# uncbiag/DeepAtlas

Hardware: AMD Instinct MI355X
Metric: training volumes/sec at 160x192x160 fp32; Dice vs CPU ref (higher is better)
Workload: dtype f32; 1 GPU; seg-only UNet_light + softmax-Dice + Adam training step, batch 2/GPU, 160x192x160 fp32 (BASELINE configs[1]); global_batch=2, n_classes=32, parallelism=dp1, matrix_precision=fp32_split, hip_graph=False, matrix_arithmetic_bits=22

## Files before the change

deepatlas_amd/_native.py:

```python
import ctypes
import os
from ctypes import c_int, c_float, c_double, c_longlong, c_size_t, c_void_p, c_char_p, POINTER

import torch

_HERE = os.path.dirname(os.path.abspath(__file__))
LIB_PATH = os.environ.get('DA_LIB') or os.path.join(_HERE, 'csrc', 'libdeepatlas_hip.so')

P = c_void_p
I = c_int
F = c_float
LL = c_longlong
SZ = c_size_t
DBL = c_double

SIGNATURES = {
    'da_version': (I, []),
    'da_device_info': (I, [POINTER(c_int), POINTER(c_int), POINTER(c_size_t), c_char_p, I]),
    'da_w_oik_to_tio': (I, [P, P, I, I, I, P]),
    'da_w_tio_to_oik': (I, [P, P, I, I, I, P]),
    'da_w_iok_to_tio': (I, [P, P, I, I, I, P]),
    'da_w_tio_to_iok': (I, [P, P, I, I, I, P]),
    'da_w_iok_flip_to_tio': (I, [P, P, I, I, I, P]),
    'da_w_tio_to_iok_flip': (I, [P, P, I, I, I, P]),
    'da_w_tio_to_oik_acc': (I, [P, P, I, I, I, P]),
    'da_w_tio_to_iok_acc': (I, [P, P, I, I, I, P]),
    'da_w_tio_to_iok_flip_acc': (I, [P, P, I, I, I, P]),
    'da_conv3d_k3_ws_bytes': (SZ, [I, I, I, I, I, I, I]),
    'da_conv3d_k3_pack_bytes': (SZ, [I, I, I, I, I, I]),
    'da_conv3d_k3_dgrad_bst': (I, [P, P, P, I, P, I, I, I, I, I, I, P, P, F, P, I, P, P, SZ, P]),
    'da_conv3d_k3_prepack': (I, [P, I, I, I, I, I, I, I, I, P, SZ, P, SZ, P, P]),
    'da_conv3d_k3_use_prepacked': (None, [P, P, SZ, P, SZ]),
    'da_conv3d_k3_prepack_many': (I, [I, P, P, P, P, P, P, P, P, P, P, P, P, P, P, P]),
    'da_conv3d_k3_fwd': (I, [P, I, P, I, P, P, P, I, I, I, I, I, I, F, P, SZ, P]),
    'da_conv3d_k3_fwd_bnstats': (I, [P, I, P, I, P, P, P, I, I, I, I, I, I, P, I, POINTER(c_int), P, SZ, P]),
    'da_conv3d_k3_dgrad': (I, [P, P, P, I, P, I, I, I, I, I, I, I, P, SZ, P]),
    'da_conv3d_k3_wgrad': (I, [P, I, P, I, P, P, P, I, I, I, I, I, I, P, SZ, P]),
    'da_conv3d_k3_fwd_pro': (I, [P, I, P, P, F, P, I, P, P, F, P, P, P, I, I, I, I, I, F, P, I, POINTER(c_int), P, SZ, P]),
    'da_conv3d_k3_wgrad_pro': (I, [P, I, P, P, F, P, I, P, P, F, P, P, I, I, I, I, I, P, SZ, P]),
    'da_upconv3d_k3_supported': (I, [I, I, I]),
    'da_upconv3d_k3_ws_bytes': (SZ, [I, I, I, I, I, I]),
    'da_upconv3d_k3_fwd': (I, [P, I, P, I, P, P, P, I, I, I, I, I, F, P, SZ, P]),
    'da_upconv3d_k3_dgrad': (I, [P, P, P, I, P, I, I, I, I, I, I, P, SZ, P]),
    'da_upconv3d_k3_wgrad': (I, [P, I, P, I, P, P, I, I, I, I, I, P, SZ, P]),
    'da_set_conv_direct': (I, [I]),
    'da_set_matrix_bf16': (I, [I]),
    'da_set_matrix_mode': (I, [I]),
    'da_pointwise_ws_bytes': (SZ, [I, I, I]),
    'da_conv1x1_fwd': (I, [P, P, P, P, LL, I, I, P, SZ, P]),
    'da_conv1x1_fwd_pro': (I, [P, P, P, F, P, P, P, LL, I, I, P, SZ, P]),
    'da_conv1x1_wgrad_pro': (I, [P, P, P, F, P, P, P, LL, I, I, P, SZ, P]),
    'da_conv1x1_dgrad': (I, [P, P, P, LL, I, I, P, SZ, P]),
    'da_conv1x1_wgrad_ws_bytes': (SZ, [LL, I, I]),
    'da_conv1x1_wgrad': (I, [P, P, P, P, LL, I, I, P, SZ, P]),
    'da_deconv_k2s2_fwd': (I, [P, P, P, P, I, I, I, I, I, I, P, SZ, P]),
    'da_deconv_k2s2_fwd_bnstats': (I, [P, P, P, P, I, I, I, I, I, I, P, I, POINTER(c_int), P, SZ, P]),
    'da_deconv_k2s2_dgrad': (I, [P, P, P, I, I, I, I, I, I, P, SZ, P]),
    'da_deconv_k2s2_bn_bwd_ws_bytes': (SZ, [I, I, I, I, I, I]),
    'da_deconv_k2s2_bn_bwd': (I, [P, P, P, P, P, P, F, P, P, P, P, P, P, P, I, I, I, I, I, I, P, I, P, SZ, P]),
    'da_deconv_k2s2_wgrad_ws_bytes': (SZ, [I, I, I, I, I, I]),
    'da_deconv_k2s2_wgrad': (I, [P, P, P, P, I, I, I, I, I, I, P, SZ, P]),
    'da_bn_ws_bytes': (SZ, [LL, I]),
    'da_bn_train_stats': (I, [P, LL, I, P, P, F, F, P, P, P, P, P, P, P, SZ, P]),
    'da_bn_train_stats_from_partials': (I, [P, I, LL, I, P, P, F, F, P, P, P, P, P, P, P]),
    'da_bn_eval_affine': (I, [P, P, P, P, F, I, P, P, P, P, P]),
    'da_bn_act_fwd': (I, [P, P, P, F, P, LL, I, P]),
    'da_bn_act_bwd': (I, [P, P, P, P, P, P, P, F, I, P, P, P, LL, I, P, SZ, P]),
    'da_bn_act_bwd_dbias': (I, [P, P, P, P, P, P, F, I, P, P, P, P, LL, I, P, SZ, P]),
    'da_bn_act_bwd_dbias_pre': (I, [P, P, P, P, P, P, F, I, P, P, P, P, LL, I, P, I, P, SZ, P]),
    'da_act_bwd': (I, [P, P, F, P, LL, P]),
    'da_act_bwd_add_dbias': (I, [P, P, P, F, P, P, LL, I, P, SZ, P]),
    'da_colsum': (I, [P, LL, I, P, P, SZ, P]),
    'da_act_bwd_add_partial': (I, [P, P, P, F, P, LL, I, P, SZ, POINTER(c_int), P]),
    'da_colsum_finish': (I, [P, I, I, P, I, P]),
    'da_maxpool2_fwd': (I, [P, P, I, I, I, I, I, P]),
    'da_maxpool2_fwd_pro': (I, [P, P, P, F, P, P, I, I, I, I, I, P]),
    'da_maxpool2_bwd': (I, [P, P, P, I, I, I, I, I, P]),
    'da_maxpool2_bwd_add': (I, [P, P, P, P, I, I, I, I, I, P]),
    'da_maxpool2_bwd_bst': (I, [P, P, P, P, I, I, I, I, I, P, F, P, I, P, P]),
    'da_upsample_nearest_fwd': (I, [P, P, I, I, I, I, I, I, I, I, P]),
    'da_upsample_nearest_bwd': (I, [P, P, I, I, I, I, I, I, I, I, P]),
    'da_warp_fwd': (I, [P, P, P, P, I, I, I, I, I, P]),
    'da_warp_bwd': (I, [P, P, P, P, P, I, I, I, I, I, P]),
    'da_label_warp_dice_ws_bytes': (SZ, [I, I]),
    'da_warp_dice_ws_bytes': (SZ, [I, I]),
    'da_warp_dice_fwd': (I, [P, P, P, I, I, I, I, I, I, I, I, F, P, P, P, SZ, P]),
    'da_softmax_dice_fwd': (I, [P, P, I, P, I, LL, I, I, I, F, P, P, P, SZ, P]),
    'da_label_warp_dice_fwd': (I, [P, I, P, I, P, I, I, I, I, I, I, I, F, P, P, P, SZ, P]),
    'da_label_warp_dice_bwd': (I, [P, I, P, I, P, P, P, P, I, I, I, I, I, P]),
    'da_softwarp_dice_ws_bytes': (SZ, [I, I]),
    'da_softwarp_dice_fwd': (I, [P, I, P, P, I, I, I, I, I, I, I, I, F, P, P, P, SZ, P]),
    'da_softwarp_dice_bwd_disp': (I, [P, I, P, P, P, P, P, I, I, I, I, I, P]),
    'da_softwarp_dice_bwd_logits': (I, [P, I, P, P, P, P, P, I, I, I, I, I, P]),
    'da_warp_adjoint_labels': (I, [P, I, P, P, P, I, I, I, I, I, P]),
    'da_seg_anat_dlogits': (I, [P, P, I, P, P, P, P, P, P, P, I, LL, I, P]),
    'da_warp_bwd_dsrc_det_ws_bytes': (SZ, [I, I, I, I, I]),
    'da_warp_bwd_dsrc_det': (I, [P, P, P, I, I, I, I, I, P, SZ, P]),
    'da_identity_grid': (I, [P, I, I, I, I, P]),
    'da_warp_labels_fwd': (I, [P, I, P, P, I, I, I, I, I, P]),
    'da_warp_labels_bwd': (I, [P, P, I, P, P, I, I, I, I, I, P]),
    'da_dice_ws_bytes': (SZ, [I, LL, I]),
    'da_dice_fwd': (I, [P, P, I, P, I, LL, I, I, I, I, F, P, P, P, SZ, P]),
    'da_dice_bwd': (I, [P, P, I, P, P, P, P, I, LL, I, I, P]),
    'da_softmax_fwd': (I, [P, P, LL, I, P]),
    'da_softmax_bwd': (I, [P, P, P, LL, I, P]),
    'da_one_hot': (I, [P, I, P, LL, I, P]),
    'da_head_dice_ws_bytes': (SZ, [I, LL, I, I]),
    'da_head_dice_fwd': (I, [P, P, P, F, P, P, P, I, I, LL, I, I, I, I, F, P, P, P, SZ, P]),
    'da_head_dice_bwd': (I, [P, P, P, F, P, P, P, I, P, P, P, P, P, I, LL, I, I, P, SZ, P]),
    'da_head_dice_bwd_bst': (I, [P, P, P, F, P, P, P, P, I, P, P, P, P, P, I, LL, I, I, P, I, P, P, SZ, P]),
# ... 218 lines not shown
```

deepatlas_amd/csrc/deconv.hip:

```cpp
#include "common.h"
#include "pointwise_internal.h"

namespace {

template <int CT>
__global__ void __launch_bounds__(256)
deconv_k2s2_fwd_kernel(const float* __restrict__ in, const float* __restrict__ w, const float* __restrict__ bias,
                       float* __restrict__ out, int N, int D, int H, int W, int Cin, int Cout) {
    const long long nvox = (long long)N * D * H * W;
    const long long v = (long long)blockIdx.x * blockDim.x + threadIdx.x;
    if (v >= nvox) return;
    const int co0 = blockIdx.y * CT;
    long long r = v;
    const int iw = (int)(r % W); r /= W;
    const int ih = (int)(r % H); r /= H;
    const int id = (int)(r % D); const int n = (int)(r / D);
    const float* x = in + v * Cin;
    const int Ho = 2 * H, Wo = 2 * W, Do = 2 * D;
#pragma unroll 1
    for (int ij = 0; ij < 4; ++ij) {
        const int i = ij >> 1, j = ij & 1;
        float acc[2][CT];
#pragma unroll
        for (int k = 0; k < 2; ++k)
// ... 153 lines not shown
static int parts_for(long long units, int O, long long* per) {
    long long parts = units < 1024 ? units : 1024;
    const long long cap = (long long)(64ull << 20) / ((long long)O * 4);
    if (parts > cap) parts = cap;
    if (parts < 1) parts = 1;
    *per = da_cdiv(units, parts);
    return (int)da_cdiv(units, *per);
}

}

extern "C" size_t da_pointwise_ws_bytes(int ntaps, int Cin, int Cout) { return da_pw_packed_bytes(ntaps, Cin, Cout) + 256; }

extern "C" int da_deconv_k2s2_fwd(const float* in, const float* w_tio, const float* bias, float* out,
                                  int N, int D, int H, int W, int Cin, int Cout, void* ws, size_t ws_bytes, void* stream) {
    if (!in || !w_tio || !out || N <= 0 || D <= 0 || H <= 0 || W <= 0 || Cin <= 0 || Cout <= 0) return DA_ERR_BADARG;
    const long long nvox = (long long)N * D * H * W;
    if (da_pw_supported(Cin, Cout))
        return da_pw_gemm(in, w_tio, 0, bias, out, nvox, D, H, W, Cin, Cout, 8, 1, 0, ws, ws_bytes, da_stream(stream));
    hipLaunchKernelGGL((deconv_k2s2_fwd_kernel<16>), dim3((unsigned)da_cdiv(nvox, 256), (unsigned)da_cdiv(Cout, 16)), dim3(256), 0, da_stream(stream),
                       in, w_tio, bias, out, N, D, H, W, Cin, Cout);
    DA_LAUNCH_CHECK();
    return 0;
}

extern "C" int da_deconv_k2s2_fwd_bnstats(const float* in, const float* w_tio, const float* bias, float* out,
                                          int N, int D, int H, int W, int Cin, int Cout,
                                          double* stats_partial, int stats_capacity, int* stats_nparts,
                                          void* ws, size_t ws_bytes, void* stream) {
    if (stats_nparts) *stats_nparts = 0;
    if (!in || !w_tio || !out || N <= 0 || D <= 0 || H <= 0 || W <= 0 || Cin <= 0 || Cout <= 0) return DA_ERR_BADARG;
    const long long nvox = (long long)N * D * H * W;
    const long long nblk = da_cdiv(nvox, 256);
    if (stats_partial && stats_nparts && da_pw_supported(Cin, Cout) && nblk <= stats_capacity) {
        const int rc = da_pw_gemm(in, w_tio, 0, bias, out, nvox, D, H, W, Cin, Cout, 8, 1, 0, ws, ws_bytes, da_stream(stream), stats_partial);
        if (rc == 0) *stats_nparts = (int)nblk;
        return rc;
    }
    return da_deconv_k2s2_fwd(in, w_tio, bias, out, N, D, H, W, Cin, Cout, ws, ws_bytes, stream);
}

extern "C" int da_deconv_k2s2_dgrad(const float* dy, const float* w_tio, float* dx,
                                    int N, int D, int H, int W, int Cin, int Cout, void* ws, size_t ws_bytes, void* stream) {
    if (!dy || !w_tio || !dx || N <= 0 || D <= 0 || H <= 0 || W <= 0 || Cin <= 0 || Cout <= 0) return DA_ERR_BADARG;
    const long long nvox = (long long)N * D * H * W;
    if (da_pw_supported(Cout, Cin))
        return da_pw_gemm(dy, w_tio, 1, nullptr, dx, nvox, D, H, W, Cout, Cin, 8, 1, 1, ws, ws_bytes, da_stream(stream));
    hipLaunchKernelGGL((deconv_k2s2_dgrad_kernel<16>), dim3((unsigned)da_cdiv(nvox, 256), (unsigned)da_cdiv(Cin, 16)), dim3(256), 0, da_stream(stream),
                       dy, w_tio, dx, N, D, H, W, Cin, Cout);
    DA_LAUNCH_CHECK();
    return 0;
}

struct BnBwdWs { size_t bn_bytes, fused_bytes; void *bn, *fused; size_t bytes; };
static BnBwdWs bn_bwd_layout(long long M, int Cin, int Cout, void* ws) {
    const size_t bn = da_bn_ws_bytes(M * 8, Cout), fused = da_deconv_bn_bwd_ws_bytes(M, Cin, Cout);
    DaCarve c(ws); return BnBwdWs{bn, fused, c.take<char>(bn), c.take<char>(fused), c.off};
}
extern "C" size_t da_deconv_k2s2_bn_bwd_ws_bytes(int N, int D, int H, int W, int Cin, int Cout) {
    return bn_bwd_layout((long long)N * D * H * W, Cin, Cout, nullptr).bytes;
}
extern "C" int da_deconv_k2s2_bn_bwd(const float* gout, const float* y, const float* mean, const float* rstd, const float* scale, const float* shift, float act_slope,
                                     const float* in, const float* w_tio, float* dx, float* dw_tio, float* dbias, float* dgamma, float* dbeta,
                                     int N, int D, int H, int W, int Cin, int Cout, const double* pre, int pre_n,
                                     void* ws, size_t ws_bytes, void* stream) {
    if (!gout || !y || !mean || !rstd || !scale || !shift || !in || !w_tio || !dx || !dw_tio || N <= 0 || D <= 0 || H <= 0 || W <= 0) return DA_ERR_BADARG;
    if (!da_deconv_bn_bwd_supported(Cin, Cout)) return DA_ERR_UNSUPPORTED;
    if (ws_bytes < da_deconv_k2s2_bn_bwd_ws_bytes(N, D, H, W, Cin, Cout)) return DA_ERR_WS_SMALL;
    const long long M = (long long)N * D * H * W;
    hipStream_t st = da_stream(stream);
    const BnBwdWs l = bn_bwd_layout(M, Cin, Cout, ws);
    const float* cm = nullptr;
    int rc = da_bn_bwd_sums(gout, y, mean, rstd, scale, shift, act_slope, M * 8, Cout, dgamma, dbeta, &cm, l.bn, l.bn_bytes, st, pre, pre_n);
    if (rc) return rc;
    return da_deconv_bn_bwd(gout, y, mean, rstd, scale, shift, cm, act_slope, in, w_tio, dx, dw_tio, dbias, M, D, H, W, Cin, Cout, l.fused, l.fused_bytes, st);
}

constexpr size_t kWgPad = 512;
static size_t wgrad_bytes(size_t direct_floats, size_t matrix_bytes, int Cout) {
    const size_t direct = da_align(direct_floats * sizeof(float));
    return (direct > matrix_bytes ? direct : matrix_bytes) + kWgPad + da_bn_ws_bytes(0, Cout);
}
static size_t k2s2_wgrad_bytes(int N, int D, int H, int W, int Cin, int Cout, int Cbias) {
    long long per;
    const int O = 8 * Cin * Cout;
    const int parts = parts_for((long long)N * D * H * W, O, &per);
    const size_t mf = da_pw_supported(Cin, Cout) ? da_pw_wgrad_ws_bytes((long long)N * D * H * W, 8, Cin, Cout) : 0;
    return wgrad_bytes((size_t)parts * O, mf, Cbias);
}
extern "C" size_t da_deconv_k2s2_wgrad_ws_bytes(int N, int D, int H, int W, int Cin, int Cout) { return k2s2_wgrad_bytes(N, D, H, W, Cin, Cout, Cout); }

extern "C" int da_deconv_k2s2_wgrad(const float* in, const float* dy, float* dw_tio, float* dbias,
                                    int N, int D, int H, int W, int Cin, int Cout,
                                    void* ws, size_t ws_bytes, void* stream) {
    if (!in || !dy || !dw_tio || N <= 0 || D <= 0 || H <= 0 || W <= 0 || Cin <= 0 || Cout <= 0) return DA_ERR_BADARG;
    if (ws_bytes < da_deconv_k2s2_wgrad_ws_bytes(N, D, H, W, Cin, Cout)) return DA_ERR_WS_SMALL;
    hipStream_t st = da_stream(stream);
    long long per;
    const int O = 8 * Cin * Cout;
    const int parts = parts_for((long long)N * D * H * W, O, &per);
    const DaColsumTail cs = da_colsum_tail(ws, da_deconv_k2s2_wgrad_ws_bytes(N, D, H, W, Cin, Cout), Cout);
    int rc_pw = DA_ERR_UNSUPPORTED;
    if (da_pw_supported(Cin, Cout)) rc_pw = da_pw_wgrad(in, dy, dw_tio, (long long)N * D * H * W, D, H, W, Cin, Cout, 8, 1, ws, cs.front, st);
    if (rc_pw != 0 && rc_pw != DA_ERR_UNSUPPORTED) return rc_pw;
    if (rc_pw == DA_ERR_UNSUPPORTED) {
        float* partial = (float*)ws;
// ... 203 lines not shown
```

deepatlas_amd/csrc/pointwise_internal.h:

```cpp
#pragma once
#include <hip/hip_runtime.h>
#include <stddef.h>

bool da_pw_supported(int K, int N);
size_t da_pw_packed_bytes(int ntaps, int K, int N);
int da_pw_gemm(const float* a, const float* w, int transposed, const float* bias, float* out,
               long long M, int D, int H, int W, int K, int N, int ntaps, int up, int gather,
               void* ws, size_t ws_bytes, hipStream_t st, double* stats_partial = nullptr,
               const float* pro_scale = nullptr, const float* pro_shift = nullptr, float pro_slope = -1.f,
               int a_bf16 = 0, int out_bf16 = 0);
size_t da_pw_wgrad_ws_bytes(long long M, int ntaps, int Cin, int Cout);
int da_pw_wgrad(const float* in, const float* dy, float* dw, long long M, int D, int H, int W, int Cin, int Cout,
                int ntaps, int up, void* ws, size_t ws_bytes, hipStream_t st,
                const float* pro_scale = nullptr, const float* pro_shift = nullptr, float pro_slope = -1.f, int in_bf16 = 0, int dy_bf16 = 0);

int da_bn_bwd_sums(const float* dy, const float* x, const float* mean, const float* rstd, const float* scale, const float* shift, float act_slope,
                   long long M, int C, float* dgamma, float* dbeta, const float** cm_out, void* ws, size_t ws_bytes, hipStream_t st, const double* pre, int pre_n);
bool da_deconv_bn_bwd_supported(int Cin, int Cout);
size_t da_deconv_bn_bwd_ws_bytes(long long M, int Cin, int Cout);
int da_deconv_bn_bwd(const float* gout, const float* y, const float* mean, const float* rstd, const float* scale, const float* shift, const float* cm, float slope,
                     const float* in, const float* w_tio, float* dx, float* dw_tio, float* dbias,
                     long long M, int D, int H, int W, int Cin, int Cout, void* ws, size_t ws_bytes, hipStream_t st);
```

deepatlas_amd/csrc/pointwise_mfma.hip:

```cpp
#include "common.h"
#include "pointwise_internal.h"

typedef float f32x4 __attribute__((ext_vector_type(4)));

namespace {

struct PwP {
    const float* a; const float* wp; const float* bias; float* out;
    long long M;
    int D, H, W;
    int K, Nc;
    int lda, ldo;
    int accum;
    int ntaps, up;
    double* stats; int stats_ld;
    const float* ps; const float* pt; float pslope;
};

__device__ __forceinline__ float pw_act01(float z, float s) { return fmaxf(z, z * s); }

__device__ __forceinline__ long long fine0(long long v, int D, int H, int W) {
    int n, d, h, w; da_vox4(v, D, H, W, n, d, h, w);
    return (((long long)n * (2 * D) + 2 * d) * (2 * H) + 2 * h) * (long long)(2 * W) + 2 * w;
}
__device__ __forceinline__ long long tapoff(int t, int H, int W) {
    return ((long long)(t >> 2) * (2 * H) + ((t >> 1) & 1)) * (2 * W) + (t & 1);
}

template <int KC, int NT, bool GATHER, bool STATS = false, typename TA = float, typename TO = float>
__global__ void __launch_bounds__(256) pw_mfma_kernel(PwP p) {
    static_assert(!(STATS && GATHER), "statistics are an epilogue of the scatter form");
    const TA* __restrict__ pa = reinterpret_cast<const TA*>(p.a);
    TO* __restrict__ po = reinterpret_cast<TO*>(p.out);
    constexpr int MT = 4;
    const int lane = threadIdx.x & 63;
    const int wave = threadIdx.x >> 6;
    const int i = lane & 15, g = lane >> 4;
    const long long vbase = ((long long)blockIdx.x * 4 + wave) * (MT * 16);
    if (!STATS && vbase >= p.M) return;
    double d1[STATS ? NT : 1], d2[STATS ? NT : 1];
#pragma unroll
    for (int n = 0; n < (STATS ? NT : 1); ++n) { d1[n] = 0.0; d2[n] = 0.0; }
    const float4* wp4 = reinterpret_cast<const float4*>(p.wp) + lane;

    long long arow[MT];
    bool aval[MT];
#pragma unroll
    for (int r = 0; r < MT; ++r) {
        const long long v = vbase + r * 16 + i;
        aval[r] = v < p.M;
        const long long vv = aval[r] ? v : 0;
        arow[r] = (GATHER && p.up) ? fine0(vv, p.D, p.H, p.W) : vv;
    }
    f32x4 acc[MT][NT];

    if constexpr (!GATHER) {
        float4 a[MT][KC];
#pragma unroll
        for (int r = 0; r < MT; ++r)
#pragma unroll
            for (int c = 0; c < KC; ++c)
                a[r][c] = aval[r] ? da_ldq(pa, (arow[r] * p.lda + 16 * c + 4 * g) >> 2) : make_float4(0.f, 0.f, 0.f, 0.f);
        if (p.ps) {
#pragma unroll
            for (int c = 0; c < KC; ++c) {
                const float4 sc = *reinterpret_cast<const float4*>(p.ps + 16 * c + 4 * g), sf = *reinterpret_cast<const float4*>(p.pt + 16 * c + 4 * g);
#pragma unroll
                for (int r = 0; r < MT; ++r) {
                    a[r][c].x = pw_act01(a[r][c].x * sc.x + sf.x, p.pslope); a[r][c].y = pw_act01(a[r][c].y * sc.y + sf.y, p.pslope);
                    a[r][c].z = pw_act01(a[r][c].z * sc.z + sf.z, p.pslope); a[r][c].w = pw_act01(a[r][c].w * sc.w + sf.w, p.pslope);
                    if constexpr (DaEl<TA>::bf) a[r][c] = da_unpack_bf16x4(da_pack_bf16x4(a[r][c]));
                }
            }
        }
        long long orow[MT][4];
#pragma unroll
        for (int r = 0; r < MT; ++r)
#pragma unroll
            for (int reg = 0; reg < 4; ++reg) {
                const long long v = vbase + r * 16 + 4 * g + reg;
                orow[r][reg] = (v < p.M) ? (p.up ? fine0(v, p.D, p.H, p.W) : v) : -1;
            }
        long long obase[MT][4];
#pragma unroll
        for (int r = 0; r < MT; ++r)
#pragma unroll
            for (int reg = 0; reg < 4; ++reg) obase[r][reg] = orow[r][reg] * p.ldo + i;
        float bv[NT];
#pragma unroll
        for (int n = 0; n < NT; ++n) bv[n] = (p.bias && !p.accum) ? p.bias[16 * n + i] : 0.f;
#pragma unroll 1
        for (int t = 0; t < p.ntaps; ++t) {
            const long long toff = p.up ? tapoff(t, p.H, p.W) : 0;
#pragma unroll
            for (int r = 0; r < MT; ++r)
#pragma unroll
                for (int n = 0; n < NT; ++n) acc[r][n] = (f32x4){bv[n], bv[n], bv[n], bv[n]};
            if (p.accum) {
#pragma unroll
                for (int r = 0; r < MT; ++r)
#pragma unroll
                    for (int reg = 0; reg < 4; ++reg) {
                        if (orow[r][reg] < 0) continue;
                        const long long o = (orow[r][reg] + toff) * p.ldo + i;
#pragma unroll
                        for (int n = 0; n < NT; ++n) acc[r][n][reg] = da_ld1(po, o + 16 * n);
                    }
// ... 5 lines not shown
                    const float4 b = wp4[(((size_t)t * NT + n) * KC + c) * 64];
#pragma unroll
                    for (int r = 0; r < MT; ++r) {
                        acc[r][n] = __builtin_amdgcn_mfma_f32_16x16x4f32(a[r][c].x, b.x, acc[r][n], 0, 0, 0);
                        acc[r][n] = __builtin_amdgcn_mfma_f32_16x16x4f32(a[r][c].y, b.y, acc[r][n], 0, 0, 0);
                        acc[r][n] = __builtin_amdgcn_mfma_f32_16x16x4f32(a[r][c].z, b.z, acc[r][n], 0, 0, 0);
                        acc[r][n] = __builtin_amdgcn_mfma_f32_16x16x4f32(a[r][c].w, b.w, acc[r][n], 0, 0, 0);
                    }
                }
            {
                TO* const pot = po + toff * p.ldo;
#pragma unroll
                for (int r = 0; r < MT; ++r)
#pragma unroll
                    for (int reg = 0; reg < 4; ++reg) {
                        if (orow[r][reg] < 0) continue;
#pragma unroll
                        for (int n = 0; n < NT; ++n) da_st1(pot, obase[r][reg] + 16 * n, acc[r][n][reg]);
                    }
            }
            if constexpr (STATS) {
#pragma unroll
                for (int n = 0; n < NT; ++n) {
                    float t1 = 0.f, t2 = 0.f;
#pragma unroll
                    for (int r = 0; r < MT; ++r)
#pragma unroll
                        for (int reg = 0; reg < 4; ++reg) {
                            const float v = (orow[r][reg] >= 0) ? acc[r][n][reg] : 0.f;
                            t1 += v; t2 += v * v;
                        }
                    d1[n] += (double)t1; d2[n] += (double)t2;
                }
            }
        }
        if constexpr (STATS) {
            __shared__ double sred[4][2][NT * 16];
#pragma unroll
            for (int n = 0; n < NT; ++n) {
                double a = d1[n], b = d2[n];
                a += __shfl_xor(a, 16); b += __shfl_xor(b, 16);
                a += __shfl_xor(a, 32); b += __shfl_xor(b, 32);
                if (g == 0) { sred[wave][0][n * 16 + i] = a; sred[wave][1][n * 16 + i] = b; }
            }
            __syncthreads();
            if ((int)threadIdx.x < NT * 16) {
                const int c = threadIdx.x;
                p.stats[((size_t)blockIdx.x * 2 + 0) * p.stats_ld + c] = (sred[0][0][c] + sred[1][0][c]) + (sred[2][0][c] + sred[3][0][c]);
                p.stats[((size_t)blockIdx.x * 2 + 1) * p.stats_ld + c] = (sred[0][1][c] + sred[1][1][c]) + (sred[2][1][c] + sred[3][1][c]);
            }
        }
    } else {
#pragma unroll
        for (int n = 0; n < NT; ++n) {
            const float bvn = (p.bias && !p.accum) ? p.bias[16 * n + i] : 0.f;
#pragma unroll
            for (int r = 0; r < MT; ++r) acc[r][n] = (f32x4){bvn, bvn, bvn, bvn};
        }
        if (p.accum) {
#pragma unroll
            for (int r = 0; r < MT; ++r)
#pragma unroll
                for (int reg = 0; reg < 4; ++reg) {
                    const long long v = vbase + r * 16 + 4 * g + reg;
                    if (v >= p.M) continue;
                    const long long o = v * p.ldo + i;
#pragma unroll
                    for (int n = 0; n < NT; ++n) acc[r][n][reg] = da_ld1(po, o + 16 * n);
                }
        }
#pragma unroll 1
        for (int t = 0; t < p.ntaps; ++t) {
            const long long toff = p.up ? tapoff(t, p.H, p.W) : 0;
#pragma unroll
            for (int c = 0; c < KC; ++c) {
                float4 a[MT];
#pragma unroll
                for (int r = 0; r < MT; ++r)
                    a[r] = aval[r] ? da_ldq(pa, ((arow[r] + toff) * p.lda + 16 * c + 4 * g) >> 2) : make_float4(0.f, 0.f, 0.f, 0.f);
#pragma unroll
                for (int n = 0; n < NT; ++n) {
                    const float4 b = wp4[(((size_t)t * NT + n) * KC + c) * 64];
#pragma unroll
                    for (int r = 0; r < MT; ++r) {
                        acc[r][n] = __builtin_amdgcn_mfma_f32_16x16x4f32(a[r].x, b.x, acc[r][n], 0, 0, 0);
                        acc[r][n] = __builtin_amdgcn_mfma_f32_16x16x4f32(a[r].y, b.y, acc[r][n], 0, 0, 0);
                        acc[r][n] = __builtin_amdgcn_mfma_f32_16x16x4f32(a[r].z, b.z, acc[r][n], 0, 0, 0);
                        acc[r][n] = __builtin_amdgcn_mfma_f32_16x16x4f32(a[r].w, b.w, acc[r][n], 0, 0, 0);
                    }
                }
            }
        }
#pragma unroll
        for (int r = 0; r < MT; ++r)
#pragma unroll
            for (int reg = 0; reg < 4; ++reg) {
                const long long v = vbase + r * 16 + 4 * g + reg;
                if (v >= p.M) continue;
                const long long o = v * p.ldo + i;
#pragma unroll
                for (int n = 0; n < NT; ++n) da_st1(po, o + 16 * n, acc[r][n][reg]);
            }
    }
}

__global__ void pw_pack_kernel(const float* __restrict__ w, float* __restrict__ wp, int ntaps, int K, int N, int transposed,
                               int Kt, int Nt, int k0, int n0) {
    const int KC = K / 16, NT = N / 16;
    const long long total = (long long)ntaps * NT * KC * 256;
    for (long long idx = (long long)blockIdx.x * blockDim.x + threadIdx.x; idx < total; idx += (long long)gridDim.x * blockDim.x) {
        const int m = (int)(idx & 3), lane = (int)((idx >> 2) & 63);
        long long rest = idx >> 8;
        const int c = (int)(rest % KC); rest /= KC;
        const int n = (int)(rest % NT); const int t = (int)(rest / NT);
        const int k = 16 * c + 4 * (lane >> 4) + m, j = 16 * n + (lane & 15);
        wp[idx] = transposed ? w[((size_t)t * Nt + n0 + j) * Kt + k0 + k] : w[((size_t)t * Kt + k0 + k) * Nt + n0 + j];
    }
}

struct PwWgP {
    const float* in; const float* dy; float* partial;
    long long M; int D, H, W, Cin, Cout, ntaps, up;
    int ldi, ldy;
    long long vox_per_wave;
    const float* ps; const float* pt; float pslope;
};

template <typename T> __device__ __forceinline__ float pw_buf_ld1(__amdgpu_buffer_rsrc_t r, unsigned byte_off) {
    if constexpr (DaEl<T>::bf) return __uint_as_float((unsigned)(unsigned short)__builtin_amdgcn_raw_buffer_load_b16(r, byte_off, 0, 0) << 16);
    else return __builtin_bit_cast(float, __builtin_amdgcn_raw_buffer_load_b32(r, byte_off, 0, 0));
}
__device__ __forceinline__ void pw_buf_ld2_bf16(__amdgpu_buffer_rsrc_t r, unsigned byte_off, float& lo, float& hi) {
    const unsigned u = (unsigned)__builtin_amdgcn_raw_buffer_load_b32(r, byte_off, 0, 0);
    lo = __uint_as_float(u << 16); hi = __uint_as_float(u & 0xFFFF0000u);
}
template <int CIT, int COT, int TPB, typename TI = float, typename TY = float>
__global__ void __launch_bounds__(256) pw_mfma_wgrad_kernel(PwWgP p) {
    constexpr unsigned EI = DaEl<TI>::bytes, EY = DaEl<TY>::bytes;
    constexpr bool PAIRI = DaEl<TI>::bf && CIT % 2 == 0, PAIRY = DaEl<TY>::bf && COT % 2 == 0;
    auto chan_i = [](int a, int m) -> int { return PAIRI ? 32 * (a >> 1) + 2 * m + (a & 1) : 16 * a + m; };
    auto chan_y = [](int c, int n) -> int { return PAIRY ? 32 * (c >> 1) + 2 * n + (c & 1) : 16 * c + n; };
    extern __shared__ __attribute__((aligned(16))) float red[];
    const int lane = threadIdx.x & 63;
    const int wave = threadIdx.x >> 6;
    const int i = lane & 15, g = lane >> 4;
    const int t0 = blockIdx.y * TPB;
    f32x4 acc[CIT][TPB][COT];
#pragma unroll
    for (int a = 0; a < CIT; ++a)
#pragma unroll
        for (int t = 0; t < TPB; ++t)
#pragma unroll
            for (int c = 0; c < COT; ++c) acc[a][t][c] = (f32x4){0.f, 0.f, 0.f, 0.f};
    long long toffs[TPB];
// ... 311 lines not shown
            for (int n = 0; n < NT; ++n)
                *reinterpret_cast<float4*>(&red2[par][wave][r * NT + n][lane * 4]) = make_float4(acc_dx[r][n][0], acc_dx[r][n][1], acc_dx[r][n][2], acc_dx[r][n][3]);
        __syncthreads();
        {
            const int r = wave / NT, n = wave % NT;
            float4 s = *reinterpret_cast<const float4*>(&red2[par][0][wave][lane * 4]);
#pragma unroll
            for (int w = 1; w < 4; ++w) { const float4 t = *reinterpret_cast<const float4*>(&red2[par][w][wave][lane * 4]); s.x += t.x; s.y += t.y; s.z += t.z; s.w += t.w; }
            const float sv[4] = {s.x, s.y, s.z, s.w};
#pragma unroll
            for (int reg = 0; reg < 4; ++reg) {
                const long long v = chunk * (MT * 16) + r * 16 + 4 * g + reg;
                if (v < p.M) p.dx[v * CIN + 16 * n + i] = sv[reg];
            }
        }
        par ^= 1;
#if defined(DA_DB_ABL) && (DA_DB_ABL & 8)
        }
#endif
        chunk = next;
#pragma unroll
        for (int r = 0; r < MT; ++r) {
            frow[r] = frow2[r]; aval[r] = aval2[r];
#pragma unroll
            for (int m = 0; m < 4; ++m)
#pragma unroll
                for (int a = 0; a < NT; ++a) ain[r][m][a] = ain2[r][m][a];
        }
    }
    float* part = p.dw_partial + (size_t)blockIdx.x * 8 * CIN * COUT;
#pragma unroll
    for (int tt = 0; tt < 2; ++tt)
#pragma unroll
        for (int a = 0; a < NT; ++a)
#pragma unroll
            for (int c = 0; c < KC; ++c)
#pragma unroll
                for (int reg = 0; reg < 4; ++reg)
                    part[((size_t)(t0 + tt) * CIN + 16 * a + 4 * g + reg) * COUT + 16 * c + i] = acc_dw[tt][a][c][reg];
    __syncthreads();
    double* cred = reinterpret_cast<double*>(&red2[0][0][0][0]);
#pragma unroll
    for (int c = 0; c < KC; ++c)
#pragma unroll
        for (int m = 0; m < 4; ++m) {
            double v = (double)colacc[c][m];
            v = pw_dpp_add_f64<0xB1>(v); v = pw_dpp_add_f64<0x4E>(v); v = pw_dpp_add_f64<0x141>(v); v = pw_dpp_add_f64<0x140>(v);
            if (i == 0) cred[wave * COUT + 16 * c + 4 * g + m] = v;
        }
    __syncthreads();
    if ((int)threadIdx.x < COUT) p.col_partial[((size_t)blockIdx.x * 2) * COUT + threadIdx.x] = (cred[threadIdx.x] + cred[COUT + threadIdx.x]) + (cred[2 * COUT + threadIdx.x] + cred[3 * COUT + threadIdx.x]);
}

template <int KC, int NT, typename TA, typename TO>
int launch_pw_t(const PwP& p, bool gather, hipStream_t st) {
    const unsigned grid = (unsigned)da_cdiv(p.M, 256);
    if (gather) hipLaunchKernelGGL((pw_mfma_kernel<KC, NT, true, false, TA, TO>), dim3(grid), dim3(256), 0, st, p);
    else if (p.stats) hipLaunchKernelGGL((pw_mfma_kernel<KC, NT, false, true, TA, TO>), dim3(grid), dim3(256), 0, st, p);
    else hipLaunchKernelGGL((pw_mfma_kernel<KC, NT, false, false, TA, TO>), dim3(grid), dim3(256), 0, st, p);
    DA_LAUNCH_CHECK();
    return 0;
}
template <int KC, int NT>
int launch_pw(const PwP& p, bool gather, hipStream_t st, int a_bf, int o_bf) {
    if (a_bf && o_bf) return launch_pw_t<KC, NT, da_bf16, da_bf16>(p, gather, st);
    if (a_bf) return launch_pw_t<KC, NT, da_bf16, float>(p, gather, st);
    if (o_bf) return launch_pw_t<KC, NT, float, da_bf16>(p, gather, st);
    return launch_pw_t<KC, NT, float, float>(p, gather, st);
}

}

bool da_pw_supported(int K, int N) {
    return K % 16 == 0 && N % 16 == 0 && K >= 16 && K <= 1024 && N >= 16 && N <= 1024;
}

size_t da_pw_packed_bytes(int ntaps, int K, int N) { return da_align((size_t)ntaps * (K < 64 ? K : 64) * (N < 64 ? N : 64) * sizeof(float)); }

int da_pw_gemm(const float* a, const float* w, int transposed, const float* bias, float* out,
               long long M, int D, int H, int W, int K, int N, int ntaps, int up, int gather,
               void* ws, size_t ws_bytes, hipStream_t st, double* stats_partial, const float* pro_scale, const float* pro_shift, float pro_slope, int a_bf, int o_bf) {
    if (!da_pw_supported(K, N)) return DA_ERR_UNSUPPORTED;
    if ((stats_partial || pro_scale) && gather) return DA_ERR_BADARG;
    if (o_bf && K > 64) return DA_ERR_UNSUPPORTED;
    if (pro_scale && (!pro_shift || pro_slope >= 1.f)) return DA_ERR_UNSUPPORTED;
    if (ws_bytes < da_pw_packed_bytes(ntaps, K, N)) return DA_ERR_WS_SMALL;
    float* wp = (float*)ws;
    for (int n0 = 0; n0 < N; n0 += 64) {
        const int nn = (N - n0) < 64 ? (N - n0) : 64;
        for (int k0 = 0; k0 < K; k0 += 64) {
            const int kk = (K - k0) < 64 ? (K - k0) : 64;
            const long long total = (long long)ntaps * kk * nn;
            hipLaunchKernelGGL(pw_pack_kernel, dim3(da_grid(total, 256, 512)), dim3(256), 0, st, w, wp, ntaps, kk, nn, transposed, K, N, k0, n0);
            DA_LAUNCH_CHECK();
            PwP p;
            p.a = reinterpret_cast<const float*>(reinterpret_cast<const char*>(a) + (size_t)k0 * (a_bf ? 2 : 4)); p.wp = wp; p.bias = bias ? bias + n0 : nullptr;
            p.out = reinterpret_cast<float*>(reinterpret_cast<char*>(out) + (size_t)n0 * (o_bf ? 2 : 4)); p.M = M; p.D = D; p.H = H; p.W = W;
            p.K = kk; p.Nc = nn; p.lda = K; p.ldo = N; p.accum = k0 > 0 ? 1 : 0; p.ntaps = ntaps; p.up = up;
            p.stats = (stats_partial && k0 + 64 >= K) ? stats_partial + n0 : nullptr; p.stats_ld = N;
            p.ps = pro_scale ? pro_scale + k0 : nullptr; p.pt = pro_scale ? pro_shift + k0 : nullptr; p.pslope = pro_slope < 0.f ? 1.f : pro_slope;
            const int KC = kk / 16, NT = nn / 16;
            int rc = DA_ERR_UNSUPPORTED;
#define DA_PW_CASE(kc, nt) if (KC == kc && NT == nt) rc = launch_pw<kc, nt>(p, gather != 0, st, a_bf, o_bf)
            DA_PW_CASE(1, 1); DA_PW_CASE(1, 2); DA_PW_CASE(2, 1); DA_PW_CASE(2, 2); DA_PW_CASE(4, 4);
            DA_PW_CASE(1, 4); DA_PW_CASE(4, 1); DA_PW_CASE(2, 4); DA_PW_CASE(4, 2);
            DA_PW_CASE(3, 3); DA_PW_CASE(1, 3); DA_PW_CASE(3, 1); DA_PW_CASE(2, 3); DA_PW_CASE(3, 2); DA_PW_CASE(3, 4); DA_PW_CASE(4, 3);
#undef DA_PW_CASE
            if (rc) return rc;
        }
    }
    return 0;
}

static int wg_blocks(long long M, size_t O, long long* vox_per_wave) {
    long long blocks = 1024;
    const long long cap = (long long)((64ull << 20) / (O * 4)); if (blocks > cap) blocks = cap < 1 ? 1 : cap;
    long long vpw = da_cdiv(M, blocks * 4);
    vpw = da_cdiv(vpw, 4) * 4;
    if (vpw < 4) vpw = 4;
    *vox_per_wave = vpw;
    return (int)da_cdiv(M, vpw * 4);
}

static size_t wg_partial_bytes(long long M, int ntaps, int Cin, int Cout) {
    const int ci[2] = {Cin < 64 ? Cin : 64, Cin % 64 ? Cin % 64 : 64}, co[2] = {Cout < 64 ? Cout : 64, Cout % 64 ? Cout % 64 : 64};
    size_t worst = 0;
    for (int a = 0; a < 2; ++a)
        for (int b = 0; b < 2; ++b) {
            long long vpw;
            const size_t O = (size_t)ntaps * ci[a] * co[b];
            const size_t bytes = da_align((size_t)wg_blocks(M, O, &vpw) * O * sizeof(float));
            if (bytes > worst) worst = bytes;
        }
    return worst;
}

struct PwWgWs { float *partial, *tmp; size_t bytes; };
static PwWgWs pw_wgrad_layout(long long M, int ntaps, int Cin, int Cout, void* ws) {
    DaCarve c(ws); return PwWgWs{(float*)c.take<char>(wg_partial_bytes(M, ntaps, Cin, Cout)), c.take<float>((size_t)ntaps * (Cin < 64 ? Cin : 64) * (Cout < 64 ? Cout : 64)), c.off};
}
size_t da_pw_wgrad_ws_bytes(long long M, int ntaps, int Cin, int Cout) { return pw_wgrad_layout(M, ntaps, Cin, Cout, nullptr).bytes; }

__global__ void pw_place_kernel(const float* __restrict__ src, float* __restrict__ dw, int ntaps, int cic, int coc, int Cin, int Cout, int ci0, int co0) {
    const int total = ntaps * cic * coc;
    for (int i = blockIdx.x * blockDim.x + threadIdx.x; i < total; i += gridDim.x * blockDim.x) {
        const int co = i % coc; const int ci = (i / coc) % cic; const int t = i / (coc * cic);
        dw[((size_t)t * Cin + ci0 + ci) * Cout + co0 + co] = src[i];
    }
}

static int g_wg_in_bf = 0, g_wg_dy_bf = 0;
template <int CIT, int COT, int TPB, typename TI, typename TY>
static int launch_pw_wgrad_t(const PwWgP& p, int nblocks, hipStream_t st) {
    const size_t shm = (size_t)CIT * TPB * COT * 64 * 4 * sizeof(float);
    return da_launch_lds<pw_mfma_wgrad_kernel<CIT, COT, TPB, TI, TY>>(dim3(nblocks, p.ntaps / TPB), dim3(256), shm, st, p);
}
// ... 119 lines not shown
```

include/deepatlas_hip.h:

```cpp
#ifndef DEEPATLAS_HIP_H
#define DEEPATLAS_HIP_H

#include <stddef.h>
#include <stdint.h>

#ifdef __cplusplus
extern "C" {
#endif

#define DA_ERR_BADARG   (-1)
#define DA_ERR_WS_SMALL (-2)
#define DA_ERR_UNSUPPORTED (-3)

int  da_version(void);
int  da_device_info(int* cu_count, int* wave_size, size_t* hbm_bytes, char* arch, int arch_len);

int da_w_oik_to_tio(const float* w_oik, float* w_tio, int Cout, int Cin, int K3, void* stream);
int da_w_tio_to_oik(const float* w_tio, float* w_oik, int Cout, int Cin, int K3, void* stream);
int da_w_iok_to_tio(const float* w_iok, float* w_tio, int Cin, int Cout, int K3, void* stream);
int da_w_tio_to_iok(const float* w_tio, float* w_iok, int Cin, int Cout, int K3, void* stream);
int da_w_iok_flip_to_tio(const float* w_iok, float* w_tio, int Cin, int Cout, int K3, void* stream);
int da_w_tio_to_iok_flip(const float* w_tio, float* w_iok, int Cin, int Cout, int K3, void* stream);
int da_w_tio_to_oik_acc(const float* w_tio, float* w_oik, int Cout, int Cin, int K3, void* stream);
int da_w_tio_to_iok_acc(const float* w_tio, float* w_iok, int Cin, int Cout, int K3, void* stream);
// ... 16 lines not shown
                       float* dw_tio, float* dbias,
                       int N, int D, int H, int W, int Cout, int stride,
                       void* ws, size_t ws_bytes, void* stream);

int da_conv3d_k3_fwd_pro(const float* in1, int C1, const float* pro1_scale, const float* pro1_shift, float pro1_slope,
                         const float* in2, int C2, const float* pro2_scale, const float* pro2_shift, float pro2_slope,
                         const float* w_tio, const float* bias, float* out,
                         int N, int D, int H, int W, int Cout, float act_slope,
                         double* stats_partial, int stats_capacity, int* stats_nparts,
                         void* ws, size_t ws_bytes, void* stream);
int da_conv3d_k3_wgrad_pro(const float* in1, int C1, const float* pro1_scale, const float* pro1_shift, float pro1_slope,
                           const float* in2, int C2, const float* pro2_scale, const float* pro2_shift, float pro2_slope,
                           const float* dy, float* dw_tio,
                           int N, int D, int H, int W, int Cout,
                           void* ws, size_t ws_bytes, void* stream);

int da_upconv3d_k3_supported(int C1, int C2, int Cout);
size_t da_upconv3d_k3_ws_bytes(int N, int Dc, int Hc, int Wc, int Cin, int Cout);
int da_upconv3d_k3_fwd(const float* s1, int C1, const float* s2, int C2, const float* w_tio, const float* bias, float* out,
                       int N, int Dc, int Hc, int Wc, int Cout, float act_slope, void* ws, size_t ws_bytes, void* stream);
int da_upconv3d_k3_dgrad(const float* dy, const float* w_tio, float* dx1, int C1, float* dx2, int C2,
                         int N, int Dc, int Hc, int Wc, int Cout, void* ws, size_t ws_bytes, void* stream);
int da_upconv3d_k3_wgrad(const float* s1, int C1, const float* s2, int C2, const float* dy, float* dw_tio,
                         int N, int Dc, int Hc, int Wc, int Cout, void* ws, size_t ws_bytes, void* stream);

int da_set_conv_direct(int on);

int da_set_matrix_bf16(int on);
int da_set_matrix_mode(int mode);

size_t da_pointwise_ws_bytes(int ntaps, int Cin, int Cout);
int da_conv1x1_fwd(const float* in, const float* w_io, const float* bias, float* out,
                   long long M, int Cin, int Cout, void* ws, size_t ws_bytes, void* stream);
int da_conv1x1_fwd_pro(const float* in, const float* pro_scale, const float* pro_shift, float pro_slope,
                       const float* w_io, const float* bias, float* out,
                       long long M, int Cin, int Cout, void* ws, size_t ws_bytes, void* stream);
int da_conv1x1_wgrad_pro(const float* in, const float* pro_scale, const float* pro_shift, float pro_slope,
                         const float* dy, float* dw_io, float* dbias,
                         long long M, int Cin, int Cout, void* ws, size_t ws_bytes, void* stream);
int da_conv1x1_dgrad(const float* dy, const float* w_io, float* dx, long long M, int Cin, int Cout,
                     void* ws, size_t ws_bytes, void* stream);
size_t da_conv1x1_wgrad_ws_bytes(long long M, int Cin, int Cout);
int da_conv1x1_wgrad(const float* in, const float* dy, float* dw_io, float* dbias,
                     long long M, int Cin, int Cout, void* ws, size_t ws_bytes, void* stream);

int da_deconv_k2s2_fwd(const float* in, const float* w_tio, const float* bias, float* out,
                       int N, int D, int H, int W, int Cin, int Cout, void* ws, size_t ws_bytes, void* stream);
int da_deconv_k2s2_fwd_bnstats(const float* in, const float* w_tio, const float* bias, float* out,
                               int N, int D, int H, int W, int Cin, int Cout,
                               double* stats_partial, int stats_capacity, int* stats_nparts,
                               void* ws, size_t ws_bytes, void* stream);
int da_deconv_k2s2_dgrad(const float* dy, const float* w_tio, float* dx,
                         int N, int D, int H, int W, int Cin, int Cout, void* ws, size_t ws_bytes, void* stream);
size_t da_deconv_k2s2_bn_bwd_ws_bytes(int N, int D, int H, int W, int Cin, int Cout);
int da_deconv_k2s2_bn_bwd(const float* gout, const float* y, const float* mean, const float* rstd, const float* scale, const float* shift, float act_slope,
                          const float* in, const float* w_tio, float* dx, float* dw_tio, float* dbias, float* dgamma, float* dbeta,
                          int N, int D, int H, int W, int Cin, int Cout, const double* pre, int pre_n,
                          void* ws, size_t ws_bytes, void* stream);
size_t da_deconv_k2s2_wgrad_ws_bytes(int N, int D, int H, int W, int Cin, int Cout);
int da_deconv_k2s2_wgrad(const float* in, const float* dy, float* dw_tio, float* dbias,
                         int N, int D, int H, int W, int Cin, int Cout,
                         void* ws, size_t ws_bytes, void* stream);

size_t da_bn_ws_bytes(long long M, int C);
int da_bn_train_stats(const float* x, long long M, int C, const float* gamma, const float* beta,
                      float eps, float momentum, float* running_mean, float* running_var,
                      float* mean, float* rstd, float* scale, float* shift,
                      void* ws, size_t ws_bytes, void* stream);
int da_bn_train_stats_from_partials(const double* partial, int nparts, long long M, int C,
                                    const float* gamma, const float* beta, float eps, float momentum,
                                    float* running_mean, float* running_var,
                                    float* mean, float* rstd, float* scale, float* shift, void* stream);
int da_bn_eval_affine(const float* gamma, const float* beta, const float* running_mean, const float* running_var,
                      float eps, int C, float* mean, float* rstd, float* scale, float* shift, void* stream);
int da_bn_act_fwd(const float* x, const float* scale, const float* shift, float act_slope, float* y,
                  long long M, int C, void* stream);
int da_bn_act_bwd(const float* dy, const float* x, const float* mean, const float* rstd, const float* gamma,
                  const float* scale, const float* shift, float act_slope, int train,
                  float* dx, float* dgamma, float* dbeta, long long M, int C,
                  void* ws, size_t ws_bytes, void* stream);
int da_bn_act_bwd_dbias(const float* dy, const float* x, const float* mean, const float* rstd,
                        const float* scale, const float* shift, float act_slope, int train,
                        float* dx, float* dgamma, float* dbeta, float* dxsum, long long M, int C,
                        void* ws, size_t ws_bytes, void* stream);
int da_bn_act_bwd_dbias_pre(const float* dy, const float* x, const float* mean, const float* rstd,
                            const float* scale, const float* shift, float act_slope, int train,
                            float* dx, float* dgamma, float* dbeta, float* dxsum, long long M, int C,
                            const double* pre, int pre_n, void* ws, size_t ws_bytes, void* stream);
int da_act_bwd(const float* dy, const float* y, float act_slope, float* dx, long long numel, void* stream);
int da_act_bwd_add_dbias(const float* g1, const float* g2, const float* y, float act_slope, float* dx, float* dbias,
                         long long M, int C, void* ws, size_t ws_bytes, void* stream);
int da_colsum(const float* x, long long M, int C, float* out, void* ws, size_t ws_bytes, void* stream);
int da_act_bwd_add_partial(const float* g1, const float* g2, const float* y, float act_slope, float* dx,
                           long long M, int C, void* partial, size_t partial_bytes, int* nparts, void* stream);
int da_colsum_finish(const void* partial, int nparts, int C, float* out, int accumulate, void* stream);

int da_maxpool2_fwd(const float* x, float* y, int N, int D, int H, int W, int C, void* stream);
int da_maxpool2_fwd_pro(const float* x, const float* pro_scale, const float* pro_shift, float pro_slope, float* act, float* y,
                        int N, int D, int H, int W, int C, void* stream);
int da_maxpool2_bwd(const float* dy, const float* x, float* dx, int N, int D, int H, int W, int C, void* stream);
int da_maxpool2_bwd_add(const float* dy, const float* x, const float* gskip, float* dx, int N, int D, int H, int W, int C, void* stream);
int da_maxpool2_bwd_bst(const float* dy, const float* x_raw, const float* gskip, float* dx, int N, int D, int H, int W, int C,
                        const float* stats4, float slope, double* bst, int bst_cap, int* bst_n, void* stream);

int da_upsample_nearest_fwd(const float* x, float* y, int N, int D, int H, int W, int C,
                            int Do, int Ho, int Wo, void* stream);
// ... 342 lines not shown
```

Before: 99.69 volumes/s.

## Add small-problem partition for gathered pointwise MFMA GEMM with split N tiles

Adds a SMALL variant of the gathered (deconv dgrad) pointwise MFMA kernel that uses fewer row tiles per wave, splits output column tiles across waves and uses 32-bit indexing. It is auto-selected when the problem is small enough that the default partition would not fill the device for several rounds. The aim is more blocks and better occupancy on the low-resolution decoder levels, at the cost of reloading A fragments per column split. A test entry point lets callers force either partition.

```diff
diff --git a/deepatlas_amd/_native.py b/deepatlas_amd/_native.py
--- a/deepatlas_amd/_native.py
+++ b/deepatlas_amd/_native.py
@@ -56,6 +56,7 @@
     'da_deconv_k2s2_fwd': (I, [P, P, P, P, I, I, I, I, I, I, P, SZ, P]),
     'da_deconv_k2s2_fwd_bnstats': (I, [P, P, P, P, I, I, I, I, I, I, P, I, POINTER(c_int), P, SZ, P]),
     'da_deconv_k2s2_dgrad': (I, [P, P, P, I, I, I, I, I, I, P, SZ, P]),
+    'da_deconv_k2s2_partition_test': (I, [I, I, P, P, P, P, I, I, I, I, I, I, P, I, POINTER(c_int), P, SZ, P]),
     'da_deconv_k2s2_bn_bwd_ws_bytes': (SZ, [I, I, I, I, I, I]),
     'da_deconv_k2s2_bn_bwd': (I, [P, P, P, P, P, P, F, P, P, P, P, P, P, P, I, I, I, I, I, I, P, I, P, SZ, P]),
     'da_deconv_k2s2_wgrad_ws_bytes': (SZ, [I, I, I, I, I, I]),
diff --git a/deepatlas_amd/csrc/deconv.hip b/deepatlas_amd/csrc/deconv.hip
--- a/deepatlas_amd/csrc/deconv.hip
+++ b/deepatlas_amd/csrc/deconv.hip
@@ -229,6 +229,26 @@
     return 0;
 }
 
+extern "C" int da_deconv_k2s2_partition_test(int op, int partition, const float* a, const float* w_tio, const float* bias, float* out,
+                                             int N, int D, int H, int W, int Cin, int Cout,
+                                             double* stats_partial, int stats_capacity, int* stats_nparts,
+                                             void* ws, size_t ws_bytes, void* stream) {
+    if (stats_nparts) *stats_nparts = 0;
+    if (!a || !w_tio || !out || N <= 0 || D <= 0 || H <= 0 || W <= 0 || Cin <= 0 || Cout <= 0 || op < 0 || op > 2) return DA_ERR_BADARG;
+    if (partition != DA_PW_PART_STREAM && partition != DA_PW_PART_SMALL) return DA_ERR_BADARG;
+    const long long nvox = (long long)N * D * H * W, nblk = da_cdiv(nvox, 256);
+    if (op == 2) {
+        if (!da_pw_supported(Cout, Cin)) return DA_ERR_UNSUPPORTED;
+        return da_pw_gemm(a, w_tio, 1, nullptr, out, nvox, D, H, W, Cout, Cin, 8, 1, 1, ws, ws_bytes, da_stream(stream), nullptr, nullptr, nullptr, -1.f, 0, 0, partition);
+    }
+    if (!da_pw_supported(Cin, Cout)) return DA_ERR_UNSUPPORTED;
+    if (op == 1 && (!stats_partial || !stats_nparts || nblk > stats_capacity)) return DA_ERR_BADARG;
+    const int rc = da_pw_gemm(a, w_tio, 0, bias, out, nvox, D, H, W, Cin, Cout, 8, 1, 0, ws, ws_bytes, da_stream(stream), op == 1 ? stats_partial : nullptr,
+                              nullptr, nullptr, -1.f, 0, 0, partition);
+    if (rc == 0 && op == 1) *stats_nparts = (int)nblk;
+    return rc;
+}
+
 struct BnBwdWs { size_t bn_bytes, fused_bytes; void *bn, *fused; size_t bytes; };
 static BnBwdWs bn_bwd_layout(long long M, int Cin, int Cout, void* ws) {
     const size_t bn = da_bn_ws_bytes(M * 8, Cout), fused = da_deconv_bn_bwd_ws_bytes(M, Cin, Cout);
diff --git a/deepatlas_amd/csrc/pointwise_internal.h b/deepatlas_amd/csrc/pointwise_internal.h
--- a/deepatlas_amd/csrc/pointwise_internal.h
+++ b/deepatlas_amd/csrc/pointwise_internal.h
@@ -8,7 +8,9 @@
                long long M, int D, int H, int W, int K, int N, int ntaps, int up, int gather,
                void* ws, size_t ws_bytes, hipStream_t st, double* stats_partial = nullptr,
                const float* pro_scale = nullptr, const float* pro_shift = nullptr, float pro_slope = -1.f,
-               int a_bf16 = 0, int out_bf16 = 0);
+               int a_bf16 = 0, int out_bf16 = 0,
+               int partition = 0);
+enum { DA_PW_PART_AUTO = 0, DA_PW_PART_STREAM = 1, DA_PW_PART_SMALL = 2 };
 size_t da_pw_wgrad_ws_bytes(long long M, int ntaps, int Cin, int Cout);
 int da_pw_wgrad(const float* in, const float* dy, float* dw, long long M, int D, int H, int W, int Cin, int Cout,
                 int ntaps, int up, void* ws, size_t ws_bytes, hipStream_t st,
diff --git a/deepatlas_amd/csrc/pointwise_mfma.hip b/deepatlas_amd/csrc/pointwise_mfma.hip
--- a/deepatlas_amd/csrc/pointwise_mfma.hip
+++ b/deepatlas_amd/csrc/pointwise_mfma.hip
@@ -1,5 +1,6 @@
 #include "common.h"
 #include "pointwise_internal.h"
+#include <type_traits>
 
 typedef float f32x4 __attribute__((ext_vector_type(4)));
 
@@ -27,32 +28,44 @@
     return ((long long)(t >> 2) * (2 * H) + ((t >> 1) & 1)) * (2 * W) + (t & 1);
 }
 
-template <int KC, int NT, bool GATHER, bool STATS = false, typename TA = float, typename TO = float>
-__global__ void __launch_bounds__(256) pw_mfma_kernel(PwP p) {
+template <int NT, bool GATHER, bool SMALL> struct PwPart {
+    static_assert(GATHER || !SMALL, "the scatter form has one partition");
+    static constexpr int MT = SMALL ? 2 : 4;
+    static constexpr int NS = (SMALL && NT % 2 == 0) ? 2 : 1;
+    static constexpr int VT = SMALL ? 2 : 4;
+    static constexpr int ROWS = VT * MT * 16;
+    static constexpr int WAVES = VT * NS;
+};
+
+template <int KC, int NT, bool GATHER, bool STATS = false, typename TA = float, typename TO = float, bool SMALL = false>
+__global__ void __launch_bounds__((64 * PwPart<NT, GATHER, SMALL>::WAVES)) pw_mfma_kernel(PwP p) {
     static_assert(!(STATS && GATHER), "statistics are an epilogue of the scatter form");
+    using PT = PwPart<NT, GATHER, SMALL>;
+    using IT = std::conditional_t<SMALL, int, long long>;
     const TA* __restrict__ pa = reinterpret_cast<const TA*>(p.a);
     TO* __restrict__ po = reinterpret_cast<TO*>(p.out);
-    constexpr int MT = 4;
+    constexpr int MT = PT::MT, NTW = NT / PT::NS;
     const int lane = threadIdx.x & 63;
-    const int wave = threadIdx.x >> 6;
+    const int wave = SMALL ? __builtin_amdgcn_readfirstlane((int)(threadIdx.x >> 6)) : (int)(threadIdx.x >> 6);
+    const int n0 = (wave / PT::VT) * NTW;
     const int i = lane & 15, g = lane >> 4;
-    const long long vbase = ((long long)blockIdx.x * 4 + wave) * (MT * 16);
+    const long long vbase = ((long long)blockIdx.x * PT::VT + wave % PT::VT) * (MT * 16);
     if (!STATS && vbase >= p.M) return;
     double d1[STATS ? NT : 1], d2[STATS ? NT : 1];
 #pragma unroll
     for (int n = 0; n < (STATS ? NT : 1); ++n) { d1[n] = 0.0; d2[n] = 0.0; }
     const float4* wp4 = reinterpret_cast<const float4*>(p.wp) + lane;
 
-    long long arow[MT];
+    IT arow[MT];
     bool aval[MT];
 #pragma unroll
     for (int r = 0; r < MT; ++r) {
         const long long v = vbase + r * 16 + i;
         aval[r] = v < p.M;
         const long long vv = aval[r] ? v : 0;
-        arow[r] = (GATHER && p.up) ? fine0(vv, p.D, p.H, p.W) : vv;
-    }
-    f32x4 acc[MT][NT];
+        arow[r] = (IT)((GATHER && p.up) ? fine0(vv, p.D, p.H, p.W) : vv);
+    }
+    f32x4 acc[MT][NTW];
 
     if constexpr (!GATHER) {
         float4 a[MT][KC];
@@ -164,8 +177,8 @@
         }
     } else {
 #pragma unroll
-        for (int n = 0; n < NT; ++n) {
-            const float bvn = (p.bias && !p.accum) ? p.bias[16 * n + i] : 0.f;
+        for (int n = 0; n < NTW; ++n) {
+            const float bvn = (p.bias && !p.accum) ? p.bias[16 * (n0 + n) + i] : 0.f;
 #pragma unroll
             for (int r = 0; r < MT; ++r) acc[r][n] = (f32x4){bvn, bvn, bvn, bvn};
         }
@@ -176,14 +189,14 @@
                 for (int reg = 0; reg < 4; ++reg) {
                     const long long v = vbase + r * 16 + 4 * g + reg;
                     if (v >= p.M) continue;
-                    const long long o = v * p.ldo + i;
-#pragma unroll
-                    for (int n = 0; n < NT; ++n) acc[r][n][reg] = da_ld1(po, o + 16 * n);
+                    const IT o = (IT)v * (IT)p.ldo + 16 * n0 + i;
+#pragma unroll
+                    for (int n = 0; n < NTW; ++n) acc[r][n][reg] = da_ld1(po, o + 16 * n);
                 }
         }
 #pragma unroll 1
         for (int t = 0; t < p.ntaps; ++t) {
-            const long long toff = p.up ? tapoff(t, p.H, p.W) : 0;
+            const IT toff = p.up ? (IT)tapoff(t, p.H, p.W) : (IT)0;
 #pragma unroll
             for (int c = 0; c < KC; ++c) {
                 float4 a[MT];
@@ -191,8 +204,8 @@
                 for (int r = 0; r < MT; ++r)
                     a[r] = aval[r] ? da_ldq(pa, ((arow[r] + toff) * p.lda + 16 * c + 4 * g) >> 2) : make_float4(0.f, 0.f, 0.f, 0.f);
 #pragma unroll
-                for (int n = 0; n < NT; ++n) {
-                    const float4 b = wp4[(((size_t)t * NT + n) * KC + c) * 64];
+                for (int n = 0; n < NTW; ++n) {
+                    const float4 b = wp4[(((size_t)t * NT + n0 + n) * KC + c) * 64];
 #pragma unroll
                     for (int r = 0; r < MT; ++r) {
                         acc[r][n] = __builtin_amdgcn_mfma_f32_16x16x4f32(a[r].x, b.x, acc[r][n], 0, 0, 0);
@@ -209,9 +222,9 @@
             for (int reg = 0; reg < 4; ++reg) {
                 const long long v = vbase + r * 16 + 4 * g + reg;
                 if (v >= p.M) continue;
-                const long long o = v * p.ldo + i;
-#pragma unroll
-                for (int n = 0; n < NT; ++n) da_st1(po, o + 16 * n, acc[r][n][reg]);
+                const IT o = (IT)v * (IT)p.ldo + 16 * n0 + i;
+#pragma unroll
+                for (int n = 0; n < NTW; ++n) da_st1(po, o + 16 * n, acc[r][n][reg]);
             }
     }
 }
@@ -629,21 +642,33 @@
     if ((int)threadIdx.x < COUT) p.col_partial[((size_t)blockIdx.x * 2) * COUT + threadIdx.x] = (cred[threadIdx.x] + cred[COUT + threadIdx.x]) + (cred[2 * COUT + threadIdx.x] + cred[3 * COUT + threadIdx.x]);
 }
 
+constexpr long long kPwSimds = 1024, kPwRoundsMin = 4;
+bool pw_small_fits(const PwP& p) {
+    const long long ld = p.lda > p.ldo ? p.lda : p.ldo;
+    return p.ntaps == 8 && p.up && p.M * 8 * ld < (1ll << 29);
+}
+bool pw_small_partition(const PwP& p) { return pw_small_fits(p) && da_cdiv(p.M, 64) < 2 * kPwRoundsMin * kPwSimds; }
+
+template <int KC, int NT, bool GATHER, bool STATS, typename TA, typename TO, bool SMALL>
+void launch_pw_k(const PwP& p, hipStream_t st) {
+    using PT = PwPart<NT, GATHER, SMALL>;
+    hipLaunchKernelGGL((pw_mfma_kernel<KC, NT, GATHER, STATS, TA, TO, SMALL>), dim3((unsigned)da_cdiv(p.M, PT::ROWS)), dim3(64 * PT::WAVES), 0, st, p);
+}
 template <int KC, int NT, typename TA, typename TO>
-int launch_pw_t(const PwP& p, bool gather, hipStream_t st) {
-    const unsigned grid = (unsigned)da_cdiv(p.M, 256);
-    if (gather) hipLaunchKernelGGL((pw_mfma_kernel<KC, NT, true, false, TA, TO>), dim3(grid), dim3(256), 0, st, p);
-    else if (p.stats) hipLaunchKernelGGL((pw_mfma_kernel<KC, NT, false, true, TA, TO>), dim3(grid), dim3(256), 0, st, p);
-    else hipLaunchKernelGGL((pw_mfma_kernel<KC, NT, false, false, TA, TO>), dim3(grid), dim3(256), 0, st, p);
+int launch_pw_t(const PwP& p, bool gather, bool small, hipStream_t st) {
+    if (gather && small) launch_pw_k<KC, NT, true, false, TA, TO, true>(p, st);
+    else if (gather) launch_pw_k<KC, NT, true, false, TA, TO, false>(p, st);
+    else if (p.stats) launch_pw_k<KC, NT, false, true, TA, TO, false>(p, st);
+    else launch_pw_k<KC, NT, false, false, TA, TO, false>(p, st);
     DA_LAUNCH_CHECK();
     return 0;
 }
 template <int KC, int NT>
-int launch_pw(const PwP& p, bool gather, hipStream_t st, int a_bf, int o_bf) {
-    if (a_bf && o_bf) return launch_pw_t<KC, NT, da_bf16, da_bf16>(p, gather, st);
-    if (a_bf) return launch_pw_t<KC, NT, da_bf16, float>(p, gather, st);
-    if (o_bf) return launch_pw_t<KC, NT, float, da_bf16>(p, gather, st);
-    return launch_pw_t<KC, NT, float, float>(p, gather, st);
+int launch_pw(const PwP& p, bool gather, bool small, hipStream_t st, int a_bf, int o_bf) {
+    if (a_bf && o_bf) return launch_pw_t<KC, NT, da_bf16, da_bf16>(p, gather, small, st);
+    if (a_bf) return launch_pw_t<KC, NT, da_bf16, float>(p, gather, small, st);
+    if (o_bf) return launch_pw_t<KC, NT, float, da_bf16>(p, gather, small, st);
+    return launch_pw_t<KC, NT, float, float>(p, gather, small, st);
 }
 
 }
@@ -656,7 +681,7 @@
 
 int da_pw_gemm(const float* a, const float* w, int transposed, const float* bias, float* out,
                long long M, int D, int H, int W, int K, int N, int ntaps, int up, int gather,
-               void* ws, size_t ws_bytes, hipStream_t st, double* stats_partial, const float* pro_scale, const float* pro_shift, float pro_slope, int a_bf, int o_bf) {
+               void* ws, size_t ws_bytes, hipStream_t st, double* stats_partial, const float* pro_scale, const float* pro_shift, float pro_slope, int a_bf, int o_bf, int partition) {
     if (!da_pw_supported(K, N)) return DA_ERR_UNSUPPORTED;
     if ((stats_partial || pro_scale) && gather) return DA_ERR_BADARG;
     if (o_bf && K > 64) return DA_ERR_UNSUPPORTED;
@@ -678,7 +703,9 @@
             p.ps = pro_scale ? pro_scale + k0 : nullptr; p.pt = pro_scale ? pro_shift + k0 : nullptr; p.pslope = pro_slope < 0.f ? 1.f : pro_slope;
             const int KC = kk / 16, NT = nn / 16;
             int rc = DA_ERR_UNSUPPORTED;
-#define DA_PW_CASE(kc, nt) if (KC == kc && NT == nt) rc = launch_pw<kc, nt>(p, gather != 0, st, a_bf, o_bf)
+            if (partition == DA_PW_PART_SMALL && !(gather && pw_small_fits(p))) return DA_ERR_UNSUPPORTED;
+            const bool small = gather && (partition == DA_PW_PART_AUTO ? pw_small_partition(p) : partition == DA_PW_PART_SMALL);
+#define DA_PW_CASE(kc, nt) if (KC == kc && NT == nt) rc = launch_pw<kc, nt>(p, gather != 0, small, st, a_bf, o_bf)
             DA_PW_CASE(1, 1); DA_PW_CASE(1, 2); DA_PW_CASE(2, 1); DA_PW_CASE(2, 2); DA_PW_CASE(4, 4);
             DA_PW_CASE(1, 4); DA_PW_CASE(4, 1); DA_PW_CASE(2, 4); DA_PW_CASE(4, 2);
             DA_PW_CASE(3, 3); DA_PW_CASE(1, 3); DA_PW_CASE(3, 1); DA_PW_CASE(2, 3); DA_PW_CASE(3, 2); DA_PW_CASE(3, 4); DA_PW_CASE(4, 3);
diff --git a/include/deepatlas_hip.h b/include/deepatlas_hip.h
--- a/include/deepatlas_hip.h
+++ b/include/deepatlas_hip.h
@@ -92,6 +92,10 @@
                                void* ws, size_t ws_bytes, void* stream);
 int da_deconv_k2s2_dgrad(const float* dy, const float* w_tio, float* dx,
                          int N, int D, int H, int W, int Cin, int Cout, void* ws, size_t ws_bytes, void* stream);
+int da_deconv_k2s2_partition_test(int op, int partition, const float* a, const float* w_tio, const float* bias, float* out,
+                                  int N, int D, int H, int W, int Cin, int Cout,
+                                  double* stats_partial, int stats_capacity, int* stats_nparts,
+                                  void* ws, size_t ws_bytes, void* stream);
 size_t da_deconv_k2s2_bn_bwd_ws_bytes(int N, int D, int H, int W, int Cin, int Cout);
 int da_deconv_k2s2_bn_bwd(const float* gout, const float* y, const float* mean, const float* rstd, const float* scale, const float* shift, float act_slope,
                           const float* in, const float* w_tio, float* dx, float* dw_tio, float* dbias, float* dgamma, float* dbeta,
```

New measurement: 100.0 volumes/s (median of 6 runs). No clear change (+0.4%).
